# mickeyjoe666/PHFPFAC

Measured on AMD Instinct MI355X. Metric: input GB/s scanned, higher is better.
Workload: dtype u8

## Files before the change

phfpfac_amd/csrc/pfac_hip.hip:

```cpp
#include <hip/hip_runtime.h>
#include <hip/hip_ext.h>

#include <stdint.h>
#include <stdio.h>
#include <stdlib.h>
#include <string.h>

#include <algorithm>
#include <mutex>
#include <type_traits>
#include <string>
#include <vector>

#include "pfac.h"

namespace {

constexpr int WAVE = 64;
constexpr int SUB = WAVE * 16;
constexpr int SUBS = 4;
constexpr int WTILE = SUB * SUBS;
constexpr int MSUBS = 2;
constexpr int MSUB = WTILE / MSUBS;
constexpr int MLANE = MSUB / WAVE;
constexpr int HALO_MAX = 1024;
constexpr int QCAP = SUB / 2 + 4 * WAVE;
#ifndef PFAC_CAPW
#define PFAC_CAPW 256
#endif
constexpr int CAPW = PFAC_CAPW;
constexpr int PACK_STATE_BITS = 20;
constexpr int MAX_WAVES_PER_BLOCK = 16;
constexpr int LDS_TOTAL = 160 * 1024;
constexpr int LDS_TABLE_MAX = 40 * 1024;

constexpr int SH_HDR = 0;
constexpr int SH_S0 = SH_HDR + 2048;
constexpr int SH_FTAB = SH_S0 + 256 * 4;
constexpr int SH_D1IDX = SH_FTAB + 4 * 256;
constexpr int SH_FIN = SH_D1IDX + 256;
constexpr int SH_COLMAP = SH_FIN + 256;
constexpr int SH_D1 = SH_COLMAP + 256;
constexpr int D1_LDS_MAX = 32 * 1024;
constexpr int D1_STATE_BITS = 20;
constexpr int D1_N2_MAX = 2048;
#ifndef PFAC_L2F_UNROLL
#define PFAC_L2F_UNROLL 1
#endif
constexpr int L2F_UNROLL = PFAC_L2F_UNROLL;
#ifndef PFAC_MASK_GATHERS
#define PFAC_MASK_GATHERS 1
#endif
constexpr bool MASK_GATHERS = PFAC_MASK_GATHERS != 0;
#ifndef PFAC_LOAD_AUX
#define PFAC_LOAD_AUX 2
#endif
constexpr int LOAD_AUX = PFAC_LOAD_AUX;
#ifndef PFAC_PAIR_DENSITY_PCT
#define PFAC_PAIR_DENSITY_PCT 40
#endif
constexpr int QDEEP = 0x8000;
constexpr int NBUF_MAX = 3;
constexpr int CAPW3_MIN = 192;
constexpr int PW_FIXED_1BUF = WTILE + QCAP * 2;
constexpr int CAPW_DENSE = 2048;
constexpr int PW_FIXED_DENSE = PW_FIXED_1BUF + CAPW_DENSE * 4;
constexpr int D2_RING = 256;
constexpr int D2_CNT_OFF = D2_RING * 8;
constexpr int D2_PREF_OFF = D2_CNT_OFF + WTILE / 2;
constexpr int D2_AUX = D2_PREF_OFF + (WTILE / 8) * 2;
static_assert(D2_AUX >= QCAP * 2 && D2_AUX % 16 == 0, "the survivor FIFO of the fallback pass lies in the same bytes");
constexpr int PW_FIXED_DENSE2 = WTILE + D2_AUX;
constexpr unsigned D2_LOG_CAP = 4096;

#ifndef PFAC_TICKET_WAYS
#define PFAC_TICKET_WAYS 4
#endif
constexpr unsigned TICKET_WAYS = PFAC_TICKET_WAYS;
constexpr unsigned CTL_WORDS = 64u * (TICKET_WAYS + 1);
constexpr unsigned SPIN_MAX = 1u << 22;
constexpr unsigned CTL_ERR = 32, CTL_OVF = 33, CTL_DONE = 34, CTL_OVF2 = 35, CTL_TOTAL = 36 ;
constexpr unsigned CTL_CURSOR = 64u * TICKET_WAYS;

typedef unsigned int u32x4 __attribute__((ext_vector_type(4)));

struct ScanArgs {
    const unsigned char *in;
    unsigned long long n_owned, n_avail;
    void *out;
    unsigned long long out_cap;
    unsigned long long *tile_index;
    unsigned chunk;
    unsigned rec_bytes;
    const int *s0;
    const int *r;
    const int2 *T;
    const int4 *T4;
    int r_words, t_entries;
    int ht_size, wbit, num_final, halo;
    int rn_bias;
    int shared_bytes, pw_bytes;
    const int *d1;
    const unsigned char *d1idx;
    const unsigned char *d1_colmap;
    const unsigned char *d1_colbyte;
    int d1_rows;
    int d1_stride, d1_ncols, d1_lds_bytes;
    const int2 *d1r2;
    int d1_n2;
    unsigned root_byte;
    int root_state;
    int l2f_mode;
    unsigned child0, child1;
// ... 228 lines not shown
    };
    if (!reached(1, false)) return;
    if (dense1) {
        unsigned col[NWALK];
        int nx[NWALK];
#pragma unroll
        for (int w = 0; w < NWALK; w++) col[w] = colmap[(win[w] >> 8) & 0xFFu];
#pragma unroll
        for (int w = 0; w < NWALK; w++) nx[w] = D1[(go[w] ? f[w] : 0u) * d1_stride + col[w]];
        if (FUSED && D1R2) {
            bool ok[NWALK];
            int2 e2[NWALK];
#pragma unroll
            for (int w = 0; w < NWALK; w++) {
                ok[w] = go[w] && nx[w] >= 0;
                e2[w] = D1R2[ok[w] ? (nx[w] >> D1_STATE_BITS) : 0];
            }
#pragma unroll
            for (int w = 0; w < NWALK; w++) {
                s[w] = ok[w] ? (nx[w] & ((1 << D1_STATE_BITS) - 1)) : -1;
                rn[w] = e2[w].x;
                cm[w] = (unsigned)e2[w].y;
            }
        } else {
#pragma unroll
            for (int w = 0; w < NWALK; w++) s[w] = go[w] ? nx[w] : -1;
        }
        k++;
    } else {
        if (FUSED && S0R) {
#pragma unroll
            for (int w = 0; w < NWALK; w++) rn[w] = S0R[win[w] & 0xFFu];
        } else {
            load_rn();
        }
        step(1);
    }
    if (!reached(2, true)) return;
    if (dense1 && !(FUSED && D1R2)) load_rn();
    step(2);
    if (!reached(3, true)) return;
    step(3);
    for (;;) {
        if (!reached(0, false)) return;
#pragma unroll
        for (int w = 0; w < NWALK; w++) {
            const unsigned p = pos[w] + 1u + k;
            const unsigned lo = t32[p >> 2], hi = t32[(p >> 2) + 1];
            win[w] = __builtin_amdgcn_alignbyte(hi, lo, p & 3u);
        }
        if (USE_CM) {
            bool any = false;
#pragma unroll
            for (int w = 0; w < NWALK; w++) {
                go[w] = go[w] && ((cm[w] >> (win[w] & 31u)) & 1u) != 0u;
                any = any || go[w];
            }
            if (!__any(any)) return;
        }
        step(0);
        if (!reached(1, true)) return;
        step(1);
        if (!reached(2, true)) return;
        step(2);
        if (!reached(3, true)) return;
        step(3);
    }
}

__device__ __forceinline__ void put_record(const ScanArgs &a, unsigned long long ri, unsigned tpos, unsigned gpos, unsigned state) {
    if (ri >= a.out_cap) return;
    if (a.rec_bytes == 2) {
        static_cast<unsigned short *>(a.out)[ri] = (unsigned short)(tpos | (state << 12));
    } else if (a.rec_bytes == 4) {
        static_cast<unsigned *>(a.out)[ri] = tpos | (state << 12);
    } else {
        pfac_record rec;
        rec.pos = gpos;
        rec.state = state;
        static_cast<pfac_record *>(a.out)[ri] = rec;
    }
}

template <bool W8, bool DIRECT>
__device__ __forceinline__ void walk_store(const ScanArgs &a, const unsigned char *tile, const int *s0, const int *R, const int2 *T,
                                           unsigned pos, unsigned lim, unsigned *stage, unsigned long long ri, unsigned gpos) {
    unsigned n = 0;
    int s = s0[tile[pos]];
    unsigned p = pos + 1;
    while (s >= 0) {
        if (s < a.num_final) {
            if (DIRECT) put_record(a, ri + n, pos, gpos, (unsigned)s);
            else if (ri + n < a.stage_cap) stage[ri + n] = pos | ((unsigned)s << 12);
            n++;
        }
        if (p >= lim) break;
        s = phf_step<W8>(R, T, s, tile[p], a.wbit, a.ht_size);
        p++;
    }
}

struct Dense1 {
    const unsigned char *colmap;
    const unsigned char *idx;
    const int *rows;
    bool on;
    const int2 *r2;
    const int *s0r;
};

template <bool W8, bool DIRECT, int NWALK, bool FUSED, int ROOT>
__device__ __forceinline__ unsigned roundN(const ScanArgs &a, const unsigned char *tile, const int *s0, const Dense1 &d1,
                                           const int *R, const int2 *T, const unsigned short *q, unsigned q0,
                                           unsigned nact, int lane, unsigned *stage, unsigned lim,
                                           unsigned long long tile_base, unsigned long long wrun) {
    static_assert(NWALK >= 1 && NWALK <= 4, "one to four walks per lane");
    constexpr int MREG = NWALK == 4 ? 4 : 2;
    bool active[NWALK], deepf[NWALK];
    unsigned pos[NWALK], n[NWALK], m[NWALK][MREG];
    bool anydeep = false;
#pragma unroll
    for (int w = 0; w < NWALK; w++) {
        active[w] = (unsigned)lane + WAVE * w < nact;
        const unsigned e = active[w] ? q[q0 + WAVE * w + lane] : 0u;
        pos[w] = e & 0xFFFu;
        deepf[w] = (e & QDEEP) != 0;
        anydeep = anydeep || deepf[w];
    }
#ifdef PFAC_ABL_NOWALK
    anydeep = false;
#endif
    if (!__any(anydeep)) {
#pragma unroll
        for (int w = 0; w < NWALK; w++) {
            if (!active[w]) continue;
            const unsigned st = ROOT == 1 ? (unsigned)a.root_state : (unsigned)s0[tile[pos[w]]];
            const unsigned long long ri = wrun + WAVE * w + lane;
            if (DIRECT) put_record(a, ri, pos[w], (unsigned)tile_base + pos[w], st);
            else if (ri < a.stage_cap) stage[ri] = pos[w] | (st << 12);
        }
        return nact;
    }
    walkN<W8, NWALK, FUSED, MREG, ROOT>(tile, s0, a.root_state, d1.idx, d1.colmap, (unsigned)a.d1_stride, d1.rows, d1.on, d1.r2, d1.s0r, R, T, a.T4, pos, active, deepf, lim,
                                        a.wbit, a.ht_size, a.num_final, a.rn_bias, ROOT != 1 && d1.on && a.sec_filter != 0, n, m);
#pragma unroll
    for (int w = 0; w < NWALK; w++) {
        const unsigned c = n[w];
        if (MREG == 4) {
            const unsigned a0 = m[w][0], a1 = m[w][1], a2 = m[w][2], a3 = m[w][3];
            m[w][0] = c >= 4u ? a3 : (c == 3u ? a2 : (c == 2u ? a1 : a0));
            m[w][1] = c >= 4u ? a2 : (c == 3u ? a1 : a0);
            m[w][2] = c >= 4u ? a1 : a0;
            m[w][3] = a0;
        } else {
            const unsigned a0 = m[w][0], a1 = m[w][1];
            m[w][0] = c >= 2u ? a1 : a0;
            m[w][1] = a0;
        }
    }
    unsigned ex[NWALK], total = 0;
#pragma unroll
    for (int w0 = 0; w0 < NWALK; w0 += 2) {
        const bool pair = w0 + 1 < NWALK;
        const unsigned packed = pair ? (n[w0] | (n[pair ? w0 + 1 : w0] << 16)) : n[w0];
        const unsigned inc = wave_incl_scan(packed);
        const unsigned last = bcast_last(inc);
        const unsigned t0 = pair ? (last & 0xFFFFu) : last;
        ex[w0] = total + (pair ? (inc & 0xFFFFu) : inc) - n[w0];
        total += t0;
        if (pair) {
            ex[w0 + 1] = total + (inc >> 16) - n[w0 + 1];
            total += last >> 16;
        }
    }
#pragma unroll
    for (int w = 0; w < NWALK; w++) {
        const bool regs = n[w] <= (unsigned)MREG;
        const unsigned gpos = (unsigned)tile_base + pos[w];
        if (DIRECT) {
            const unsigned long long ri = wrun + ex[w];
            if (regs && n[w] > 0) put_record(a, ri, pos[w], gpos, m[w][0]);
#pragma unroll
            for (int k = 1; k < MREG; k++)
                if (regs && n[w] > (unsigned)k) put_record(a, ri + k, pos[w], gpos, m[w][k]);
            if (!regs) walk_store<W8, true>(a, tile, s0, R, T, pos[w], lim, nullptr, ri, gpos);
        } else {
            const unsigned ri = (unsigned)wrun + ex[w];
            if (regs && n[w] > 0 && ri < a.stage_cap) stage[ri] = pos[w] | (m[w][0] << 12);
#pragma unroll
            for (int k = 1; k < MREG; k++)
                if (regs && n[w] > (unsigned)k && ri + k < a.stage_cap) stage[ri + k] = pos[w] | (m[w][k] << 12);
            if (!regs) walk_store<W8, false>(a, tile, s0, R, T, pos[w], lim, stage, ri, 0);
        }
    }
    return total;
}

template <bool W8, bool DIRECT, int NWALK, bool FUSED, int ROOT>
__device__ __forceinline__ unsigned long long tile_pass(const ScanArgs &a, const unsigned char *tile, const int *s0,
                                                        const Dense1 &d1, const int *R, const int2 *T, unsigned short *q,
                                                        unsigned *stage, const unsigned (&keep)[MSUBS],
                                                        const unsigned (&deep)[MSUBS], int lane,
                                                        unsigned lim, unsigned long long tile_base,
                                                        unsigned long long wrun) {
    unsigned head = 0, tail = 0;
    static_assert(MSUBS == 2, "the packed scan assumes 2 half-tiles");
    const unsigned c0 = __popc(keep[0]), c1 = __popc(keep[1]);
    const unsigned pa = wave_incl_scan(c0 | (c1 << 16));
    const unsigned incls[MSUBS] = {pa & 0xFFFFu, pa >> 16};
    const unsigned cnts[MSUBS] = {c0, c1};
    const unsigned la = bcast_last(pa);
    const unsigned totals[MSUBS] = {la & 0xFFFFu, la >> 16};
    if (ROOT == 1 && !__any((deep[0] | deep[1]) != 0u)) {
        const unsigned st = (unsigned)a.root_state;
#pragma unroll
        for (int j = 0; j < MSUBS; j++) {
            if (totals[j] == 0) continue;
            const unsigned lpos = j * MSUB + lane * MLANE;
            unsigned o = (j ? totals[0] : 0u) + incls[j] - cnts[j];
#ifdef PFAC_ABL_NOSTAGE
            if (true) continue;
#endif
            if (!DIRECT && totals[0] + totals[1] <= a.stage_cap) {
                const unsigned w0 = lpos | (st << 12);
                for (unsigned m = keep[j]; m;) {
                    stage[o] = w0 + (unsigned)__ffs(m) - 1u;
                    m &= m - 1;
                    if (m) stage[o + 1] = w0 + (unsigned)__ffs(m) - 1u;
                    m &= m - 1;
                    o += 2;
                }
                continue;
            }
            for (unsigned m = keep[j]; m; m &= m - 1) {
                const unsigned pos = lpos + (__ffs(m) - 1);
                if (DIRECT) put_record(a, wrun + o, pos, (unsigned)tile_base + pos, st);
                else if (o < a.stage_cap) stage[o] = pos | (st << 12);
                o++;
            }
        }
        return wrun + totals[0] + totals[1];
    }
    constexpr unsigned RW = WAVE * NWALK;
#ifdef PFAC_TRACE_BUILD
    unsigned long long tp_round = 0, tp_n = 0, tp_t0 = __builtin_amdgcn_s_memrealtime();
#define TP_ROUND(call) do { const unsigned long long t_ = __builtin_amdgcn_s_memrealtime(); call; tp_round += __builtin_amdgcn_s_memrealtime() - t_; tp_n++; } while (0)
#else
#define TP_ROUND(call) do { call; } while (0)
#endif
#pragma unroll
    for (int j = 0; j < MSUBS; j++) {
        const unsigned mask = keep[j];
        const unsigned dmask = deep[j];
        const unsigned cnt = cnts[j];
        const unsigned incl = incls[j];
        const unsigned S = totals[j];
        if (S == 0) continue;
        const unsigned lpos = j * MSUB + lane * MLANE;
        const int ngrp = S > 512u ? 4 : 1;
        for (int gi = 0; gi < ngrp; gi++) {
            unsigned gbase = 0, gcnt = S;
            bool mine = true;
            if (ngrp != 1) {
                gbase = gi ? __builtin_amdgcn_readlane(incl, 16 * gi - 1) : 0u;
                gcnt = __builtin_amdgcn_readlane(incl, 16 * gi + 15) - gbase;
                mine = (lane >> 4) == gi;
            }
            if (tail + gcnt > (unsigned)QCAP) {
                const unsigned rem = tail - head;
                unsigned short v[NWALK];
#pragma unroll
                for (int w = 0; w < NWALK; w++) v[w] = (unsigned)lane + WAVE * w < rem ? q[head + WAVE * w + lane] : (unsigned short)0;
                wave_lds_sync();
#pragma unroll
                for (int w = 0; w < NWALK; w++) if ((unsigned)lane + WAVE * w < rem) q[WAVE * w + lane] = v[w];
                head = 0;
                tail = rem;
            }
            if (mine) {
                unsigned o = tail + (incl - cnt) - gbase;
                for (unsigned m = mask; m; m &= m - 1) {
                    const unsigned b = __ffs(m) - 1;
                    q[o++] = (unsigned short)((lpos + b) | (((dmask >> b) & 1u) << 15));
                }
            }
            tail += gcnt;
            wave_lds_sync();
            for (; head + RW <= tail; head += RW)
                TP_ROUND((wrun += roundN<W8, DIRECT, NWALK, FUSED, ROOT>(a, tile, s0, d1, R, T, q, head, RW, lane, stage, lim, tile_base, wrun)));
        }
    }
    if (tail > head) {
        if (NWALK == 2 && !DIRECT && tail - head <= (unsigned)WAVE)
            TP_ROUND((wrun += roundN<W8, DIRECT, 1, FUSED, ROOT>(a, tile, s0, d1, R, T, q, head, tail - head, lane, stage, lim, tile_base, wrun)));
        else
            TP_ROUND((wrun += roundN<W8, DIRECT, NWALK, FUSED, ROOT>(a, tile, s0, d1, R, T, q, head, tail - head, lane, stage, lim, tile_base, wrun)));
    }
#ifdef PFAC_TRACE_BUILD
    if (!DIRECT && a.dbg && blockIdx.x < 8 && lane == 0 && (threadIdx.x >> 6) == 0) {
        unsigned long long *acc = a.dbg + (size_t)blockIdx.x * 64 * 32 + 10;
        acc[0] += tp_round; acc[1] += tp_n; acc[2] += __builtin_amdgcn_s_memrealtime() - tp_t0; acc[3] += 1; acc[4] += tail - head;
    }
#endif
    return wrun;
}

template <bool SPARSE>
__device__ __forceinline__ void copy_out(const ScanArgs &a, const unsigned *stage, unsigned cnt, unsigned long long base, int lane) {
    if (cnt == 0) return;
#ifdef PFAC_ABL_NOEMIT
    return;
#endif
    if (a.rec_bytes == 2) {
        unsigned short *out = static_cast<unsigned short *>(a.out);
        if (base + cnt > a.out_cap) {
            for (unsigned i = (unsigned)lane; i < cnt; i += WAVE)
                if (base + i < a.out_cap) out[base + i] = (unsigned short)stage[i];
            return;
        }
        unsigned head = (0u - (unsigned)base) & 7u;
        head = head < cnt ? head : cnt;
        if ((unsigned)lane < head) out[base + lane] = (unsigned short)stage[lane];
        unsigned i = head + 8u * (unsigned)lane;
        for (; i + 8u <= cnt; i += 8u * WAVE) {
            const u32x4 v = {(stage[i] & 0xFFFFu) | (stage[i + 1] << 16), (stage[i + 2] & 0xFFFFu) | (stage[i + 3] << 16),
                             (stage[i + 4] & 0xFFFFu) | (stage[i + 5] << 16), (stage[i + 6] & 0xFFFFu) | (stage[i + 7] << 16)};
            __builtin_nontemporal_store(v, reinterpret_cast<u32x4 *>(out + base + i));
        }
        const unsigned tail = head + ((cnt - head) & ~7u);
        if (tail + (unsigned)lane < cnt) out[base + tail + lane] = (unsigned short)stage[tail + lane];
        return;
    }
    if (SPARSE && cnt <= 2u * WAVE && base + cnt <= a.out_cap) {
        unsigned *out = static_cast<unsigned *>(a.out);
        const unsigned v0 = (unsigned)lane < cnt ? stage[lane] : 0u, v1 = (unsigned)lane + WAVE < cnt ? stage[lane + WAVE] : 0u;
        if ((unsigned)lane < cnt) __builtin_nontemporal_store(v0, out + base + lane);
        if ((unsigned)lane + WAVE < cnt) __builtin_nontemporal_store(v1, out + base + lane + WAVE);
        return;
    }
    unsigned *out = static_cast<unsigned *>(a.out);
    if (base + cnt > a.out_cap) {
        for (unsigned i = (unsigned)lane; i < cnt; i += WAVE)
            if (base + i < a.out_cap) out[base + i] = stage[i];
        return;
    }
    unsigned head = (0u - (unsigned)base) & 3u;
    head = head < cnt ? head : cnt;
    if ((unsigned)lane < head) out[base + lane] = stage[lane];
    unsigned i = head + 4u * (unsigned)lane;
    for (; i + 4u <= cnt; i += 4u * WAVE) {
        const u32x4 v = {stage[i], stage[i + 1], stage[i + 2], stage[i + 3]};
        __builtin_nontemporal_store(v, reinterpret_cast<u32x4 *>(out + base + i));
    }
    const unsigned tail = head + ((cnt - head) & ~3u);
    if (tail + (unsigned)lane < cnt) out[base + tail + lane] = stage[tail + lane];
}

#ifndef PFAC_D2_FB
#define PFAC_D2_FB 2
#endif
#ifndef PFAC_D2_NS
#define PFAC_D2_NS 2
#endif
constexpr int D2_FB = PFAC_D2_FB;
static_assert(D2_RING >= (D2_FB + 1) * WAVE, "ring: one trip's pushes on top of a batch of left-overs");
template <bool W8>
__device__ __forceinline__ unsigned dense2_tile(const ScanArgs &a, const unsigned char *tile, const unsigned *t0, const Dense1 &d1,
                                                unsigned char *aux, unsigned *logg, int lane, unsigned lim, unsigned own_end) {
    constexpr int NS = PFAC_D2_NS;
    uint2 *ring = reinterpret_cast<uint2 *>(aux);
    const unsigned *t32 = reinterpret_cast<const unsigned *>(tile);
    const int sub = a.wbit - 8;
    const unsigned nfin = (unsigned)a.num_final, logcap = a.d2log_cap;
    const __amdgpu_buffer_rsrc_t lrs = __builtin_amdgcn_make_buffer_rsrc(logg, 0, (int)(logcap * 4u), 0x00020000);
    unsigned pos[NS], pn[NS], jn[NS];
    int s[NS], idx[NS];
    bool alive[NS];
#pragma unroll
    for (int w = 0; w < NS; w++) { pos[w] = pn[w] = jn[w] = 0u; s[w] = -1; idx[w] = 0; alive[w] = false; }
    unsigned P0 = 0, head = 0, fcount = 0, lc = 0;
    unsigned jmax = 0;
    const unsigned no_root = 0xFFFFu | ((unsigned)(a.d1_rows * a.d1_stride) << 16);
    auto lane_rank = [&](unsigned long long b) -> unsigned {
        return __builtin_amdgcn_mbcnt_hi((unsigned)(b >> 32), __builtin_amdgcn_mbcnt_lo((unsigned)b, 0u));
    };
    unsigned *stg = reinterpret_cast<unsigned *>(aux + D2_CNT_OFF);
    constexpr unsigned STG = (unsigned)(WTILE / 2 / 4);
    static_assert(STG >= (unsigned)(WAVE + 2 * D2_FB * WAVE) && STG >= (unsigned)(WAVE + PFAC_D2_NS * WAVE), "log staging: < 64 words pending + what a trip / a step adds");
    unsigned fl = 0;
    auto log_put = [&](bool f, unsigned word) {
        const unsigned long long b = __builtin_amdgcn_ballot_w64(f);
        if (b) {
            if (f) stg[(lc + lane_rank(b)) & (STG - 1u)] = word;
            lc += (unsigned)__popcll(b);
        }
// ... 329 lines not shown
        for (int i = tid; i < 256; i += blockDim.x) { d1idx_l[i] = 0; colmap_l[i] = 0; }
    }
    if (a.d1_rows > 0)
        for (int i = tid; i < a.d1_stride; i += blockDim.x) d1_l[a.d1_rows * a.d1_stride + i] = -1;
    const unsigned *t0_l = reinterpret_cast<const unsigned *>(smem + a.sh_t0);
    if (FUSED && NW == 4 && a.sh_t0)
        for (int i = tid; i < 256; i += blockDim.x) {
            const int v = a.s0[i];
            reinterpret_cast<unsigned *>(smem + a.sh_t0)[i] = v >= 0 ? (((unsigned)v < (unsigned)a.num_final ? (unsigned)v : 0xFFFFu) | ((unsigned)(a.d1idx[i] * a.d1_stride) << 16))
                                                                     : (0xFFFFu | ((unsigned)(a.d1_rows * a.d1_stride) << 16));
        }
    int2 *d1r2_l = reinterpret_cast<int2 *>(smem + SH_D1 + a.d1_lds_bytes);
    if (FUSED && a.d1_n2 > 0)
        for (int i = tid; i <= a.d1_n2; i += blockDim.x) {
            const int2 e = i < a.d1_n2 ? a.d1r2[i] : make_int2(-a.rn_bias, 0);
            d1r2_l[i] = make_int2(e.x + a.rn_bias, e.y);
        }
    int *s0r_l = reinterpret_cast<int *>(smem + SH_D1);
    const bool have_s0r = FUSED && a.d1_rows == 0;
    if (have_s0r)
        for (int i = tid; i < 256; i += blockDim.x) {
            const int v = a.s0[i];
            s0r_l[i] = v >= 0 ? a.r[v >> (a.wbit - 8)] + a.rn_bias : 0;
        }
    const Dense1 d1 = {colmap_l, d1idx_l, d1_l, a.d1_rows > 0, (FUSED && a.d1_n2 > 0) ? d1r2_l : nullptr, have_s0r ? s0r_l : nullptr};
    const int sh_tab = SH_D1 + a.d1_lds_bytes;
    const int *R = a.r;
    const int2 *T = a.T;
    if (TLDS) {
        int *lr = reinterpret_cast<int *>(smem + sh_tab);
        int2 *lt = reinterpret_cast<int2 *>(smem + sh_tab + ((a.r_words * 4 + 15) & ~15));
        for (int i = tid; i < a.r_words; i += blockDim.x) lr[i] = a.r[i];
        for (int i = tid; i < a.t_entries; i += blockDim.x) lt[i] = a.T[i];
        R = lr;
        T = lt;
    }
    const unsigned char *bm2l = smem + a.sh_bm2;
    if (a.l2f_mode == 2) {
        const unsigned *src = reinterpret_cast<const unsigned *>(a.bm2 + (ROOT == 1 ? (a.root_byte & 0xFFu) * 32u : 0u));
        unsigned *dst = reinterpret_cast<unsigned *>(smem + a.sh_bm2);
        for (int i = tid; i < a.bm2_rows * 8; i += blockDim.x) dst[i] = src[i];
    }
    __syncthreads();
#ifdef PFAC_TRACE_BUILD
    if (a.dbg && blockIdx.x < 8 && threadIdx.x == 0) a.dbg[((size_t)blockIdx.x * 64 + 1) * 32 + 15] = __builtin_amdgcn_s_memrealtime();
#endif

#ifdef PFAC_ABL_NOCOORD
    if (wave == nc) return;
#endif
    if (wave == nc) {
        __builtin_amdgcn_s_setprio(3);
#ifdef PFAC_ABL_STATIC
        unsigned abl_seq = 0;
        auto ticket = [&]() -> unsigned { return (abl_seq++) * gridDim.x + blockIdx.x; };
#else
        auto ticket = [&]() -> unsigned {
            unsigned g = 0;
            if (lane == 0) g = atomicAdd(&a.ctl[(blockIdx.x % a.ticket_ways) * 64u], 1u) * a.ticket_ways + blockIdx.x % a.ticket_ways;
            return g;
        };
#endif
        auto publish_batch = [&](unsigned r, unsigned g_lane0) -> unsigned {
            if (lane == 0) {
                lds_store(&hdr[H_ARRIVED + (r & 7)], 0u);
                lds_store(&hdr[H_BATCH + (r & 7)], g_lane0);
                __builtin_amdgcn_fence(__ATOMIC_RELEASE, "workgroup");
                lds_store(&hdr[H_EPOCH + (r & 7)], r + 1);
            }
            return __builtin_amdgcn_readfirstlane(g_lane0);
        };
        unsigned g[AHEAD];
#pragma unroll
        for (int k = 0; k < AHEAD; k++) g[k] = publish_batch((unsigned)k, ticket());
        unsigned t_pending = ticket();
        unsigned long long *cursor = reinterpret_cast<unsigned long long *>(a.ctl + CTL_CURSOR);
        auto order_chunk = [&]() -> unsigned long long {
            unsigned long long v = 0;
            if (lane == 0 && a.chunk) v = __hip_atomic_fetch_add(cursor, (unsigned long long)a.chunk, __ATOMIC_RELAXED, __HIP_MEMORY_SCOPE_AGENT);
            return v;
        };
        unsigned long long ch_base = 0, spare = order_chunk(), local_total = 0;
        unsigned ch_size = 0, ch_used = 0;
        for (unsigned r = 0;; r++) {
            const unsigned g_cur = g[0];
            const unsigned long long first = (unsigned long long)g_cur * (unsigned)nc;
            if (first >= a.n_tiles) break;
            const unsigned g_new = publish_batch(r + AHEAD, t_pending);
            t_pending = ticket();
#ifdef PFAC_TRACE_BUILD
            const bool trace = a.dbg && blockIdx.x < 8 && r < 64 && lane == 0;
            unsigned long long *tr = a.dbg + ((size_t)blockIdx.x * 64 + (r & 63)) * 32;
#endif
            PFAC_STAMP(trace, 0);
            const unsigned long long left = a.n_tiles - first;
            const unsigned n_valid = left < (unsigned long long)nc ? (unsigned)left : (unsigned)nc;
            if (!lds_wait_eq(&hdr[H_ARRIVED + (r & 7)], n_valid, err, 4u)) break;
            PFAC_STAMP(trace, 1);
            const unsigned c_raw = (unsigned)lane < n_valid ? hdr[H_CNT + (r & 7) * 16 + lane] : 0u;
            const unsigned c_all = c_raw & 0x7FFFFFFFu;
            const bool self_placed = (c_raw >> 31) != 0u;
            const unsigned c = self_placed ? 0u : c_all;
            const unsigned incl = wave_incl_scan(c);
            const unsigned tot = bcast_last(incl);
            const unsigned excl = incl - c;
            const unsigned tot_all = __any(self_placed) ? bcast_last(wave_incl_scan(c_all)) : tot;
            unsigned long long wb;
            if (tot == 0) {
                wb = ch_base + ch_used;
            } else if (tot > a.chunk) {
                unsigned long long v = 0;
                if (lane == 0) v = __hip_atomic_fetch_add(cursor, (unsigned long long)tot, __ATOMIC_RELAXED, __HIP_MEMORY_SCOPE_AGENT);
                const unsigned lo = __builtin_amdgcn_readfirstlane((unsigned)v), hi = __builtin_amdgcn_readfirstlane((unsigned)(v >> 32));
                wb = (((unsigned long long)hi << 32) | lo) + excl;
            } else if (ch_used + tot <= ch_size) {
                wb = ch_base + ch_used + excl;
                ch_used += tot;
            } else {
                const unsigned long long fits = __ballot(ch_used + incl <= ch_size);
                const unsigned k = (unsigned)__popcll(fits);
                const unsigned off = __builtin_amdgcn_readlane(excl, k);
                const unsigned lo = __builtin_amdgcn_readfirstlane((unsigned)spare), hi = __builtin_amdgcn_readfirstlane((unsigned)(spare >> 32));
                const unsigned long long nb = ((unsigned long long)hi << 32) | lo;
                wb = (unsigned)lane < k ? ch_base + ch_used + excl : nb + (excl - off);
                ch_base = nb;
                ch_size = a.chunk;
                ch_used = tot - off;
                spare = order_chunk();
            }
            local_total += tot_all;
            const bool mute = (a.fault & 1u) && blockIdx.x == 1 && r == 1;
            if (lane < nc) {
                hdr[H_WBASE + (r & 7) * 32 + lane * 2] = (unsigned)wb;
                hdr[H_WBASE + (r & 7) * 32 + lane * 2 + 1] = (unsigned)(wb >> 32);
            }
            __builtin_amdgcn_fence(__ATOMIC_RELEASE, "workgroup");
            if (lane == 0 && !mute) lds_store(&hdr[H_READY + (r & 7)], r + 1);
            if ((unsigned)lane < n_valid && !self_placed) a.tile_index[first + (unsigned)lane] = wb | ((unsigned long long)c << TIX_CNT_SHIFT);
#ifdef PFAC_TRACE_BUILD
            if (trace) { tr[2] = __builtin_amdgcn_s_memrealtime(); tr[3] = g_cur; }
#endif
#pragma unroll
            for (int k = 0; k + 1 < AHEAD; k++) g[k] = g[k + 1];
            g[AHEAD - 1] = g_new;
        }
        if (lane == 0) {
            if (local_total) __hip_atomic_fetch_add(reinterpret_cast<unsigned long long *>(a.ctl + CTL_TOTAL), local_total, __ATOMIC_RELAXED, __HIP_MEMORY_SCOPE_AGENT);
            const unsigned ovf = lds_load(&hdr[H_OVF]);
            if (ovf) __hip_atomic_fetch_add(&a.ctl[CTL_OVF], ovf, __ATOMIC_RELAXED, __HIP_MEMORY_SCOPE_AGENT);
            const unsigned ovf2 = lds_load(&hdr[H_OVF2]);
            if (ovf2) __hip_atomic_fetch_add(&a.ctl[CTL_OVF2], ovf2, __ATOMIC_RELAXED, __HIP_MEMORY_SCOPE_AGENT);
        }
        return;
    }

    unsigned char *tile = smem + a.shared_bytes + wave * a.pw_bytes;
    unsigned short *q = reinterpret_cast<unsigned short *>(tile + WTILE + a.halo);
    const bool d2 = NW == 4 && FUSED && a.dense2 != 0;
    unsigned char *aux = tile + WTILE + a.halo;
    unsigned *stage0 = reinterpret_cast<unsigned *>(aux + QCAP * 2);
    unsigned *d2log = d2 ? a.d2log + ((size_t)blockIdx.x * (unsigned)nc + (unsigned)wave) * a.d2log_cap : nullptr;
    const bool root_final = ROOT == 1 && (unsigned)a.root_state < (unsigned)a.num_final;

    u32x4 wA[SUBS], wB[SUBS];
    u32x4 hA = {0u, 0u, 0u, 0u}, hB = {0u, 0u, 0u, 0u};
    auto issue_loads = [&](unsigned long long tt, u32x4 (&w)[SUBS], u32x4 &hw) {
        const unsigned long long tb = tt * WTILE;
        const unsigned long long remain = a.n_avail - tb;
        const unsigned lm = remain < (unsigned long long)(WTILE + a.halo) ? (unsigned)remain : (unsigned)(WTILE + a.halo);
        const __amdgpu_buffer_rsrc_t rsrc = __builtin_amdgcn_make_buffer_rsrc(
            const_cast<unsigned char *>(a.in + tb), 0, (int)(lm & ~15u), 0x00020000);
#pragma unroll
        for (int j = 0; j < SUBS; j++) w[j] = __builtin_amdgcn_raw_buffer_load_b128(rsrc, j * SUB + lane * 16, 0, LOAD_AUX);
        if (lane * 16 < a.halo) hw = __builtin_amdgcn_raw_buffer_load_b128(rsrc, WTILE + lane * 16, 0, 0);
    };
    auto probe = [&](unsigned rr, unsigned long long &tt) -> bool {
#ifdef PFAC_ABL_NOCOORD
        tt = ((unsigned long long)rr * gridDim.x + blockIdx.x) * (unsigned)nc + (unsigned)wave;
        return tt < a.n_tiles;
#endif
        if (!lds_wait_eq(&hdr[H_EPOCH + (rr & 7)], rr + 1, err, 16u)) return false;
        tt = (unsigned long long)__builtin_amdgcn_readfirstlane(hdr[H_BATCH + (rr & 7)]) * (unsigned)nc + (unsigned)wave;
        return tt < a.n_tiles;
    };
    auto record_base = [&](unsigned rr, unsigned long long &base) -> bool {
        if (!lds_wait_eq(&hdr[H_READY + (rr & 7)], rr + 1, err, 8u)) return false;
        const unsigned blo = __builtin_amdgcn_readfirstlane(hdr[H_WBASE + (rr & 7) * 32 + wave * 2]);
        const unsigned bhi = __builtin_amdgcn_readfirstlane(hdr[H_WBASE + (rr & 7) * 32 + wave * 2 + 1]);
        base = ((unsigned long long)bhi << 32) | blo;
        return true;
    };

    unsigned r = 0;
    unsigned long long t = 0, t_n1 = 0;
    bool have_n1 = false;
    if (!probe(0, t)) return;
    issue_loads(t, wA, hA);
    if (LOAD_DEPTH == 2) {
        have_n1 = probe(1, t_n1);
        if (have_n1) issue_loads(t_n1, wB, hB);
    }

    constexpr int LAG_MAX = NB - 1;
    const unsigned nbuf = NB == 3 ? 3u : a.nbuf;
    const unsigned lag = NB == 3 ? 2u : a.nbuf - 1u;
    bool pend_have[LAG_MAX];
    unsigned pend_cnt[LAG_MAX], buf = 0;
#pragma unroll
    for (int k = 0; k < LAG_MAX; k++) { pend_have[k] = false; pend_cnt[k] = 0; }

    auto round_body = [&](u32x4 (&w)[SUBS], u32x4 &hw) -> bool {
        const unsigned long long tile_base = t * WTILE;
        const unsigned long long remain = a.n_avail - tile_base;
        const unsigned lim = remain < (unsigned long long)(WTILE + a.halo) ? (unsigned)remain : (unsigned)(WTILE + a.halo);

#ifdef PFAC_TRACE_BUILD
        const bool trace = a.dbg && blockIdx.x < 8 && r < 64 && lane == 0 && wave == 0;
        unsigned long long *tr = a.dbg + ((size_t)blockIdx.x * 64 + (r & 63)) * 32;
#endif
        PFAC_STAMP(trace, 4);
#ifndef PFAC_ABL_NOLDSCOPY
// ... 74 lines not shown
                deep[j] = m1 & nextc;
                keep[j] = root_final ? m1 : deep[j];
            } else {
                unsigned dm = 0, fm = 0;
                const unsigned *t32 = reinterpret_cast<const unsigned *>(tile);
                unsigned cand = m1;
                if (ROOT != 1 && a.sec_filter) {
                    const unsigned nx = *reinterpret_cast<const unsigned *>(tile + off + 32);
                    const unsigned s32 = ((unsigned)ftab[nx & 0xFFu] >> 4) & 1u;
                    cand = m1 & ((((rlo >> 16) | (rhi & 0xFFFF0000u)) >> 1) | (s32 << 31));
                }
#ifdef PFAC_ABL_NOCLASS
                cand = 0;
#endif
                if (ROOT != 1 && a.l2f_mode == 3) {
                    dm = cand;
                    cand = 0;
                }
                for (unsigned mm = cand; mm;) {
                    unsigned b[L2F_UNROLL], win[L2F_UNROLL], v[L2F_UNROLL], fin[L2F_UNROLL];
                    bool on[L2F_UNROLL];
#pragma unroll
                    for (int u = 0; u < L2F_UNROLL; u++) {
                        on[u] = mm != 0u;
                        b[u] = on[u] ? (unsigned)__ffs(mm) - 1u : 0u;
                        mm &= mm - 1u;
                        const unsigned p = off + b[u];
                        const unsigned lo = t32[p >> 2], hi = t32[(p >> 2) + 1];
                        win[u] = __builtin_amdgcn_alignbyte(hi, lo, p & 3u);
                    }
#pragma unroll
                    for (int u = 0; u < L2F_UNROLL; u++) {
                        const unsigned b0 = win[u] & 0xFFu, b1 = (win[u] >> 8) & 0xFFu;
                        v[u] = bm2l[(ROOT == 1 ? 0u : b0 * 32u) + (b1 >> 3)];
                        fin[u] = ROOT == 1 ? 0u : (unsigned)finl[b0];
                    }
#pragma unroll
                    for (int u = 0; u < L2F_UNROLL; u++) {
                        const unsigned b1 = (win[u] >> 8) & 0xFFu;
                        dm |= on[u] ? ((v[u] >> (b1 & 7u)) & 1u) << b[u] : 0u;
                        fm |= on[u] ? fin[u] << b[u] : 0u;
                    }
                }
                deep[j] = dm;
                keep[j] = dm | (ROOT == 1 ? (root_final ? m1 : 0u) : fm);
            }
#ifdef PFAC_TRACE_BUILD
            asm volatile("" :: "v"(keep[j]), "v"(deep[j]));
            PFAC_STAMP(trace && r > 0 && j == 0, 13);
#endif
        }
        }

#ifdef PFAC_ABL_NOKEEP
        asm volatile("" :: "v"(keep[0]), "v"(keep[1]), "v"(deep[0]), "v"(deep[1]));
        keep[0] = keep[1] = deep[0] = deep[1] = 0;
#endif
        PFAC_STAMP(trace, 6);
        const unsigned long long cnt = d2done ? (unsigned long long)d2cnt : !__any((keep[0] | keep[1]) != 0u) ? 0ull :
            tile_pass<W8, false, NW, FUSED, ROOT>(a, tile, s0, d1, R, T, q, stage, keep, deep, lane, lim, tile_base, 0);
        PFAC_STAMP(trace, 7);
#ifdef PFAC_TRACE_BUILD
        if (a.dbg && blockIdx.x < 8 && r < 64 && lane == 0) tr[16 + wave] = __builtin_amdgcn_s_memrealtime();
#endif
        const bool overflow = cnt > a.stage_cap;
        const bool now = overflow || nbuf == 1;
        unsigned arrival = 0;
#ifdef PFAC_ABL_NOCOORD
        if (false)
#endif
        if (lane == 0) {
            hdr[H_CNT + (r & 7) * 16 + wave] = (unsigned)cnt | ((now && cnt != 0) ? 0x80000000u : 0u);
            if (cnt > a.small_cap) {
                atomicAdd(&hdr[H_OVF2], 1u);
                if (cnt > a.sparse_cap) atomicAdd(&hdr[H_OVF], 1u);
            }
            __builtin_amdgcn_fence(__ATOMIC_RELEASE, "workgroup");
            arrival = atomicAdd(&hdr[H_ARRIVED + (r & 7)], 1u);
        }
        if (__builtin_amdgcn_readfirstlane(arrival) * 2u >= (unsigned)nc) __builtin_amdgcn_s_setprio(1);
        else __builtin_amdgcn_s_setprio(0);

        if (now && cnt != 0) {
            unsigned long long v = 0;
            if (lane == 0)
                v = __hip_atomic_fetch_add(reinterpret_cast<unsigned long long *>(a.ctl + CTL_CURSOR), (unsigned long long)cnt,
                                           __ATOMIC_RELAXED, __HIP_MEMORY_SCOPE_AGENT);
            const unsigned long long base = ((unsigned long long)__builtin_amdgcn_readfirstlane((unsigned)(v >> 32)) << 32) |
                                            __builtin_amdgcn_readfirstlane((unsigned)v);
            if (lane == 0) a.tile_index[t] = base | ((unsigned long long)cnt << TIX_CNT_SHIFT);
            PFAC_STAMP(trace && r > 0 && d2, 13);
            if (NW == 4 && FUSED && d2done) {
                dense2_scatter(a, aux, d2log, (unsigned)cnt, base, lane);
                PFAC_STAMP(trace && r > 0, 14);
            }
            else if (overflow)
                tile_pass<W8, true, NW, FUSED, ROOT>(a, tile, s0, d1, R, T, q, stage, keep, deep, lane, lim, tile_base, base);
            else
                copy_out<!TLDS>(a, stage, (unsigned)cnt, base, lane);
        }
        if (NB == 2) emit_pending(pend_have[0], pend_cnt[0]);
        PFAC_STAMP(trace, 8);
        if (NB == 3) { pend_have[LAG_MAX - 1] = pend_have[0]; pend_cnt[LAG_MAX - 1] = pend_cnt[0]; }
        pend_have[0] = !now; pend_cnt[0] = (unsigned)cnt;
        buf = buf + 1u >= nbuf ? 0u : buf + 1u;
        if (LOAD_DEPTH == 1) {
            if (!more_far) return false;
            t = t_far;
        } else {
            if (!have_n1) return false;
            t = t_n1;
            t_n1 = t_far;
            have_n1 = more_far;
        }
        r++;
        return true;
    };
    for (;;) {
        if (!round_body(wA, hA)) break;
        if (LOAD_DEPTH == 2 && !round_body(wB, hB)) break;
    }
#pragma unroll
    for (int k = LAG_MAX - 1; k >= 0; k--) {
        if ((unsigned)k < lag && pend_have[k] && pend_cnt[k] != 0) {
            unsigned long long base = 0;
            if (record_base(r - (unsigned)k, base))
                copy_out<!TLDS>(a, stage0 + ((buf + nbuf - 1u - (unsigned)k) % nbuf) * a.stage_cap, pend_cnt[k], base, lane);
        }
    }
}

template <bool TLDS, bool W8, int ROOT, bool FUSED, int NW, int NB = 2>
__global__ __launch_bounds__(WAVE * MAX_WAVES_PER_BLOCK) void pfac_scan_kernel(ScanArgs a) {
    static_assert(NB == 2 || (NB == 3 && NW <= 3), "three staging buffers: the sparse-mode kernels (dense mode has one)");
    static_assert(!(TLDS && FUSED), "the fused table is for tables gathered through L2");
    static_assert(NW == (TLDS ? 1 : 2) || (FUSED && (NW == 3 || NW == 4)), "walks per lane: 1 (LDS tables), 2 (L2 tables), 3 (L2, fused), 4 (L2, fused, dense matches)");
    extern __shared__ __attribute__((aligned(16))) unsigned char smem[];
    const ErrCh err = {&a.ctl[CTL_ERR], a.spin_max};
#ifdef PFAC_TRACE_BUILD
    if (a.dbg && blockIdx.x < 8 && threadIdx.x == 0) a.dbg[((size_t)blockIdx.x * 64 + 0) * 32 + 15] = __builtin_amdgcn_s_memrealtime();
#endif
    scan_body<TLDS, W8, ROOT, FUSED, NW, NB>(a, smem, err);
    unsigned *hdr = reinterpret_cast<unsigned *>(smem + SH_HDR);
    if ((threadIdx.x & (WAVE - 1)) == 0) {
        asm volatile("s_waitcnt vmcnt(0)" ::: "memory");
        const unsigned left = atomicAdd(&hdr[H_EXIT], 1u);
        if (left + 1 == (blockDim.x >> 6)) {
#ifdef PFAC_TRACE_BUILD
            if (a.dbg && blockIdx.x < 8) a.dbg[((size_t)blockIdx.x * 64 + 2) * 32 + 15] = __builtin_amdgcn_s_memrealtime();
#endif
            const unsigned done = __hip_atomic_fetch_add(&a.ctl[CTL_DONE], 1u, __ATOMIC_ACQ_REL, __HIP_MEMORY_SCOPE_AGENT);
            if (done + 1 == gridDim.x) {
                const unsigned long long tot = __hip_atomic_load(reinterpret_cast<unsigned long long *>(a.ctl + CTL_TOTAL), __ATOMIC_RELAXED, __HIP_MEMORY_SCOPE_AGENT);
                const unsigned long long cur = __hip_atomic_load(reinterpret_cast<unsigned long long *>(a.ctl + CTL_CURSOR), __ATOMIC_RELAXED, __HIP_MEMORY_SCOPE_AGENT);
                a.res[0] = (unsigned)tot; a.res[1] = (unsigned)(tot >> 32);
                a.res[2] = __hip_atomic_load(&a.ctl[CTL_ERR], __ATOMIC_RELAXED, __HIP_MEMORY_SCOPE_AGENT);
                a.res[3] = __hip_atomic_load(&a.ctl[CTL_OVF], __ATOMIC_RELAXED, __HIP_MEMORY_SCOPE_AGENT);
                a.res[4] = (unsigned)cur; a.res[5] = (unsigned)(cur >> 32);
                a.res[6] = __hip_atomic_load(&a.ctl[CTL_OVF2], __ATOMIC_RELAXED, __HIP_MEMORY_SCOPE_AGENT);
            }
        }
    }
}


__global__ void pfac_repack_kernel(const int *blob, int *s0, int *r, int2 *T, int *idmap, int max_row, int ht_size,
                                   int num_final, int state_num, int width, int *bad) {
    const int *b_s0 = blob + PFAC_BLOB_HEADER_WORDS;
    const int *b_r = b_s0 + 256;
// ... 1690 lines not shown
    const uint64_t n_tiles = (n_owned + WTILE - 1) / WTILE;
    if (s.pending) HIP_TRY(ctx, hipStreamSynchronize(s.stream));
    s.last_cap = capacity;
    s.scanned = true;
    s.pending = true;
    for (int i = 0; i < 7; i++) s.h_ctl[i] = 0;
    const bool dense = ctx->dense && ctx->stage_cap_d;
    const StageLayout &L = ctx->sparse();
    const int wpb = dense ? ctx->waves_per_block_d : L.waves_per_block;
    const int lds_bytes = dense ? ctx->lds_bytes_d : L.lds_bytes;
    s.last_dense = dense;
    s.last_tiles = n_tiles;
    s.last_owned = n_owned;
    s.last_avail = n_avail;
    s.scan_seq++;
    s.last_table = ctx->table_gen;
    s.last_rec_bytes = ctx->rec_bytes;
    s.last_records = d_records;
    rc = ensure_ctl(ctx, s);
    if (rc) return rc;
    rc = ensure_tiles(ctx, s, n_tiles + 1);
    if (rc) return rc;
    const uint64_t n_batches = (n_tiles + wpb - 2) / (wpb - 1);
    unsigned *const cur = s.d_ctlbuf[s.flip], *const nxt = s.d_ctlbuf[1 - s.flip];
    if (n_tiles > 0 && !s.clean[s.flip]) HIP_TRY(ctx, hipMemsetAsync(cur, 0, CTL_REGION, s.stream));
    if (n_tiles == 0) HIP_TRY(ctx, hipEventRecord(s.ev0, s.stream));
    if (n_tiles > 0) {
        ScanArgs a;
        a.in = in; a.n_owned = n_owned; a.n_avail = n_avail;
        a.out = d_records; a.out_cap = capacity;
        a.tile_index = s.d_tile_index;
        a.rec_bytes = (unsigned)ctx->rec_bytes;
        a.l2f_mode = ctx->l2f_mode; a.child0 = ctx->child0; a.child1 = ctx->child1; a.n_child = ctx->n_child;
        a.bm2 = ctx->d_bm2; a.bm2_rows = ctx->bm2_rows; a.sh_bm2 = ctx->sh_bm2; a.sh_t0 = ctx->sh_t0;
        a.sec2 = ctx->d_bm2 + 256 * 32; a.sec_filter = ctx->sec_filter;
        a.spin_max = ctx->spin_max; a.fault = ctx->fault;
        a.s0 = ctx->d_s0; a.r = ctx->d_r; a.T = ctx->d_T; a.T4 = ctx->d_T4_alloc; a.rn_bias = ctx->rn_bias;
        a.r_words = ctx->max_row; a.t_entries = ctx->ht_size;
        a.ht_size = ctx->ht_size; a.wbit = ctx->width_bit; a.num_final = ctx->num_final;
        a.halo = ctx->halo;
        a.shared_bytes = ctx->shared_bytes; a.pw_bytes = dense ? ctx->pw_bytes_d : L.pw_bytes;
        a.d1 = ctx->d_d1; a.d1_rows = ctx->d1_rows; a.d1_stride = ctx->d1_stride; a.d1_ncols = ctx->d1_ncols; a.d1_lds_bytes = ctx->d1_lds_bytes;
        a.d1_colmap = ctx->d_d1 ? reinterpret_cast<const unsigned char *>(ctx->d_d1) + d1_off_col(ctx->d1_rows) : nullptr;
        a.d1_colbyte = a.d1_colmap ? a.d1_colmap + 256 : nullptr;
        a.d1_n2 = ctx->d1_n2;
        a.d1r2 = ctx->d1_n2 ? reinterpret_cast<const int2 *>(reinterpret_cast<const unsigned char *>(ctx->d_d1) + d1_off_r2(ctx->d1_rows))
                            : nullptr;
        a.d1idx = ctx->d_d1 ? reinterpret_cast<const unsigned char *>(ctx->d_d1) + (size_t)ctx->d1_rows * 1024 : nullptr;
        a.root_byte = ctx->root_byte;
        a.root_state = ctx->root_state;
        a.stage_cap = dense ? ctx->stage_cap_d : L.stage_cap;
        a.nbuf = dense ? 1u : (unsigned)L.nbuf;
        a.dense2 = dense && ctx->dense2 ? 1 : 0;
        a.d2log = nullptr; a.d2log_cap = ctx->d2log_cap;
        if (a.dense2) {
            a.stage_cap = 0;
            const size_t words = (size_t)ctx->grid_blocks * (size_t)(wpb - 1) * ctx->d2log_cap;
            if (s.d2log_words < words) {
                if (s.d_d2log) { HIP_TRY(ctx, hipStreamSynchronize(s.stream)); HIP_TRY(ctx, hipFree(s.d_d2log)); s.d_d2log = nullptr; s.d2log_words = 0; }
                HIP_TRY(ctx, hipMalloc((void **)&s.d_d2log, words * 4));
                s.d2log_words = words;
            }
            a.d2log = s.d_d2log;
        }
        a.sparse_cap = ctx->lay[0].stage_cap;
        a.small_cap = ctx->lag2_ok ? ctx->lay[1].stage_cap : ctx->lay[0].stage_cap;
        a.n_tiles = (unsigned)n_tiles;
        a.ctl = cur;
        a.zero_next = reinterpret_cast<uint4 *>(nxt);
        a.zero_vec = (unsigned)(CTL_REGION / 16);
        a.res = s.d_res;
        a.dbg = nullptr;
#ifdef PFAC_TRACE_BUILD
        if (!ctx->trace_file.empty()) {
            if (!s.d_dbg) HIP_TRY(ctx, hipMalloc((void **)&s.d_dbg, 8 * 64 * 32 * 8));
            HIP_TRY(ctx, hipMemsetAsync(s.d_dbg, 0, 8 * 64 * 32 * 8, s.stream));
            a.dbg = s.d_dbg;
        }
#endif
        const uint64_t want = n_batches;
        uint64_t grid = (uint64_t)ctx->grid_blocks < want ? (uint64_t)ctx->grid_blocks : want;
        a.ticket_ways = grid < TICKET_WAYS ? (unsigned)grid : TICKET_WAYS;
        if (ctx->ticket_ways_knob >= 1 && ctx->ticket_ways_knob < a.ticket_ways) a.ticket_ways = ctx->ticket_ways_knob;
        uint64_t chunk = (capacity / (32 * grid)) & ~3ull;
        if (chunk > (1u << 22)) chunk = 1u << 22;
        a.chunk = (chunk >= 1024 && !dense) ? (unsigned)chunk : 0u;
        void *kargs[] = {&a};
        HIP_TRY(ctx, hipExtLaunchKernel(dense ? ctx->kernel_d : (ctx->lag2 ? ctx->kernel3 : ctx->kernel), dim3((unsigned)grid),
                                        dim3(WAVE * wpb), kargs, (size_t)lds_bytes, s.stream, s.ev0, s.ev1, 0));
        s.clean[s.flip] = false;
        s.clean[1 - s.flip] = true;
        s.flip = 1 - s.flip;
    }
    if (n_tiles == 0) HIP_TRY(ctx, hipEventRecord(s.ev1, s.stream));
    return PFAC_OK;
}

int pfac_scan_finish(pfac_ctx *ctx, int slot, uint64_t *n_matches) {
    int rc = check_slot(ctx, slot);
    if (rc) return rc;
    Slot &s = ctx->slots[slot];
    if (!s.scanned) return fail(ctx, PFAC_E_STATE, "pfac_scan_finish without a scan");
    USE_DEVICE(ctx);
    HIP_TRY(ctx, hipEventSynchronize(s.ev1));
    s.pending = false;
    const uint64_t total = ((uint64_t)s.h_ctl[1] << 32) | s.h_ctl[0];
    s.last_total = total;
    s.last_used = ((uint64_t)s.h_ctl[5] << 32) | s.h_ctl[4];
    if (n_matches) *n_matches = total;
#ifdef PFAC_TRACE_BUILD
    if (s.d_dbg && !ctx->trace_file.empty()) {
        std::vector<unsigned long long> h(8 * 64 * 32);
        if (hipMemcpy(h.data(), s.d_dbg, h.size() * 8, hipMemcpyDeviceToHost) == hipSuccess) {
            if (FILE *f = fopen(ctx->trace_file.c_str(), "wb")) { fwrite(h.data(), 8, h.size(), f); fclose(f); }
        }
    }
#endif
    if (s.h_ctl[2] != 0) {
        s.clean[0] = s.clean[1] = false;
        return fail(ctx, PFAC_E_INTERNAL, "scan kernel reported a timeout (flags " + std::to_string(s.h_ctl[2]) +
                                          ": 4 arrivals, 8 record base, 16 batch ring)");
    }
    if (ctx->dense_forced < 0 && ctx->stage_cap_d && s.last_tiles >= 64) {
        const uint64_t ovf = s.h_ctl[3];
        if (!ctx->dense && ovf * 4 > s.last_tiles) ctx->dense = true;
        else if (ctx->dense && ovf * 16 < s.last_tiles) ctx->dense = false;
    }
    if (ctx->lag2_ok && !ctx->lag_forced && s.last_tiles >= 64) {
        const uint64_t ovf2 = s.h_ctl[6];
        if (ctx->lag2 && ovf2 * 16 > s.last_tiles) ctx->lag2 = false;
        else if (!ctx->lag2 && ovf2 * 64 < s.last_tiles) ctx->lag2 = true;
    }
    if (s.last_used > s.last_cap)
        return fail(ctx, PFAC_E_OVERFLOW, "record array too small: " + std::to_string(total) + " matches need " +
                                              std::to_string(s.last_used) + " records of capacity (pfac_scan_capacity_hint)");
    return PFAC_OK;
}

int pfac_scan_elapsed_ms(pfac_ctx *ctx, int slot, float *ms) {
    int rc = check_slot(ctx, slot);
    if (rc) return rc;
    if (!ms) return fail(ctx, PFAC_E_ARG, "null argument");
    Slot &s = ctx->slots[slot];
    if (!s.scanned) return fail(ctx, PFAC_E_STATE, "no scan to time");
    HIP_TRY(ctx, hipEventSynchronize(s.ev1));
    HIP_TRY(ctx, hipEventElapsedTime(ms, s.ev0, s.ev1));
    return PFAC_OK;
}

static int ensure_gsum(pfac_ctx *ctx, Slot &s, unsigned n_groups) {
    if ((uint64_t)n_groups + 1 <= s.gsum_cap) return PFAC_OK;
    if (s.d_gsum) { HIP_TRY(ctx, hipStreamSynchronize(s.stream)); HIP_TRY(ctx, hipFree(s.d_gsum)); s.d_gsum = nullptr; }
    const uint64_t cap = n_groups < 4096 ? 4097 : (uint64_t)n_groups + n_groups / 4 + 1;
    HIP_TRY(ctx, hipMalloc((void **)&s.d_gsum, cap * 8));
    s.gsum_cap = cap;
    return PFAC_OK;
}

static int expand_records(pfac_ctx *ctx, Slot &s, const void *src, uint64_t first, uint64_t n, pfac_record *d_out) {
    if (s.pending) return fail(ctx, PFAC_E_STATE, "records requested before pfac_scan_finish");
    if (first + n > s.last_total) return fail(ctx, PFAC_E_ARG, "records [first, first + n) exceed the scan's match count");
    if (s.last_used > s.last_cap) return fail(ctx, PFAC_E_OVERFLOW, "the slot's last scan overflowed its record heap: scan again with a larger one");
    if (n == 0 || s.last_tiles == 0) return PFAC_OK;
    const unsigned n_groups = (unsigned)((s.last_tiles + XGROUP - 1) / XGROUP);
    int rc = ensure_gsum(ctx, s, n_groups);
    if (rc) return rc;
    const unsigned gblocks = (n_groups + 3) / 4;
// ... 673 lines not shown
```

Before: 4915.

## Stage 16-bit records in LDS and emit them with aligned 16-byte nontemporal stores

When the output record size is 2 bytes and the single-walk path is used, matches are staged in LDS as 16-bit values instead of 32-bit words. Each tile's output allocation is rounded up to a multiple of 8 records, so copy_out can write 8 records per lane with 16-byte nontemporal stores. The ticket/placement logic pads per-tile counts and keeps the true match totals separately. The aim is to cut LDS footprint and global store instructions for the output, at the cost of padding gaps in the output buffer and more complex count bookkeeping.

```diff
diff --git a/phfpfac_amd/csrc/pfac_hip.hip b/phfpfac_amd/csrc/pfac_hip.hip
--- a/phfpfac_amd/csrc/pfac_hip.hip
+++ b/phfpfac_amd/csrc/pfac_hip.hip
@@ -29,6 +29,7 @@
 #define PFAC_CAPW 256
 #endif
 constexpr int CAPW = PFAC_CAPW;
+static_assert(CAPW % 8 == 0, "staging buffers start on 16-byte boundaries (copy_out reads them 16 bytes per lane)");
 constexpr int PACK_STATE_BITS = 20;
 constexpr int MAX_WAVES_PER_BLOCK = 16;
 constexpr int LDS_TOTAL = 160 * 1024;
@@ -423,7 +424,13 @@
     }
 }
 
-template <bool W8, bool DIRECT>
+template <bool S16>
+__device__ __forceinline__ void stage_put(const ScanArgs &a, unsigned *stage, unsigned i, unsigned v) {
+    if (S16 && a.rec_bytes == 2) reinterpret_cast<unsigned short *>(stage)[i] = (unsigned short)v;
+    else stage[i] = v;
+}
+
+template <bool W8, bool DIRECT, bool S16>
 __device__ __forceinline__ void walk_store(const ScanArgs &a, const unsigned char *tile, const int *s0, const int *R, const int2 *T,
                                            unsigned pos, unsigned lim, unsigned *stage, unsigned long long ri, unsigned gpos) {
     unsigned n = 0;
@@ -432,7 +439,7 @@
     while (s >= 0) {
         if (s < a.num_final) {
             if (DIRECT) put_record(a, ri + n, pos, gpos, (unsigned)s);
-            else if (ri + n < a.stage_cap) stage[ri + n] = pos | ((unsigned)s << 12);
+            else if (ri + n < a.stage_cap) stage_put<S16>(a, stage, (unsigned)ri + n, pos | ((unsigned)s << 12));
             n++;
         }
         if (p >= lim) break;
@@ -450,7 +457,7 @@
     const int *s0r;
 };
 
-template <bool W8, bool DIRECT, int NWALK, bool FUSED, int ROOT>
+template <bool W8, bool DIRECT, int NWALK, bool FUSED, int ROOT, bool S16>
 __device__ __forceinline__ unsigned roundN(const ScanArgs &a, const unsigned char *tile, const int *s0, const Dense1 &d1,
                                            const int *R, const int2 *T, const unsigned short *q, unsigned q0,
                                            unsigned nact, int lane, unsigned *stage, unsigned lim,
@@ -478,7 +485,7 @@
             const unsigned st = ROOT == 1 ? (unsigned)a.root_state : (unsigned)s0[tile[pos[w]]];
             const unsigned long long ri = wrun + WAVE * w + lane;
             if (DIRECT) put_record(a, ri, pos[w], (unsigned)tile_base + pos[w], st);
-            else if (ri < a.stage_cap) stage[ri] = pos[w] | (st << 12);
+            else if (ri < a.stage_cap) stage_put<S16>(a, stage, (unsigned)ri, pos[w] | (st << 12));
         }
         return nact;
     }
@@ -524,14 +531,14 @@
 #pragma unroll
             for (int k = 1; k < MREG; k++)
                 if (regs && n[w] > (unsigned)k) put_record(a, ri + k, pos[w], gpos, m[w][k]);
-            if (!regs) walk_store<W8, true>(a, tile, s0, R, T, pos[w], lim, nullptr, ri, gpos);
+            if (!regs) walk_store<W8, true, S16>(a, tile, s0, R, T, pos[w], lim, nullptr, ri, gpos);
         } else {
             const unsigned ri = (unsigned)wrun + ex[w];
-            if (regs && n[w] > 0 && ri < a.stage_cap) stage[ri] = pos[w] | (m[w][0] << 12);
+            if (regs && n[w] > 0 && ri < a.stage_cap) stage_put<S16>(a, stage, ri, pos[w] | (m[w][0] << 12));
 #pragma unroll
             for (int k = 1; k < MREG; k++)
-                if (regs && n[w] > (unsigned)k && ri + k < a.stage_cap) stage[ri + k] = pos[w] | (m[w][k] << 12);
-            if (!regs) walk_store<W8, false>(a, tile, s0, R, T, pos[w], lim, stage, ri, 0);
+                if (regs && n[w] > (unsigned)k && ri + k < a.stage_cap) stage_put<S16>(a, stage, ri + k, pos[w] | (m[w][k] << 12));
+            if (!regs) walk_store<W8, false, S16>(a, tile, s0, R, T, pos[w], lim, stage, ri, 0);
         }
     }
     return total;
@@ -545,6 +552,7 @@
                                                         unsigned lim, unsigned long long tile_base,
                                                         unsigned long long wrun) {
     unsigned head = 0, tail = 0;
+    constexpr bool S16 = NWALK == 1;
     static_assert(MSUBS == 2, "the packed scan assumes 2 half-tiles");
     const unsigned c0 = __popc(keep[0]), c1 = __popc(keep[1]);
     const unsigned pa = wave_incl_scan(c0 | (c1 << 16));
@@ -564,6 +572,17 @@
 #endif
             if (!DIRECT && totals[0] + totals[1] <= a.stage_cap) {
                 const unsigned w0 = lpos | (st << 12);
+                if (S16 && a.rec_bytes == 2) {
+                    unsigned short *s16 = reinterpret_cast<unsigned short *>(stage);
+                    for (unsigned m = keep[j]; m;) {
+                        s16[o] = (unsigned short)(w0 + (unsigned)__ffs(m) - 1u);
+                        m &= m - 1;
+                        if (m) s16[o + 1] = (unsigned short)(w0 + (unsigned)__ffs(m) - 1u);
+                        m &= m - 1;
+                        o += 2;
+                    }
+                    continue;
+                }
                 for (unsigned m = keep[j]; m;) {
                     stage[o] = w0 + (unsigned)__ffs(m) - 1u;
                     m &= m - 1;
@@ -576,7 +595,7 @@
             for (unsigned m = keep[j]; m; m &= m - 1) {
                 const unsigned pos = lpos + (__ffs(m) - 1);
                 if (DIRECT) put_record(a, wrun + o, pos, (unsigned)tile_base + pos, st);
-                else if (o < a.stage_cap) stage[o] = pos | (st << 12);
+                else if (o < a.stage_cap) stage_put<S16>(a, stage, o, pos | (st << 12));
                 o++;
             }
         }
@@ -628,14 +647,14 @@
             tail += gcnt;
             wave_lds_sync();
             for (; head + RW <= tail; head += RW)
-                TP_ROUND((wrun += roundN<W8, DIRECT, NWALK, FUSED, ROOT>(a, tile, s0, d1, R, T, q, head, RW, lane, stage, lim, tile_base, wrun)));
+                TP_ROUND((wrun += roundN<W8, DIRECT, NWALK, FUSED, ROOT, S16>(a, tile, s0, d1, R, T, q, head, RW, lane, stage, lim, tile_base, wrun)));
         }
     }
     if (tail > head) {
         if (NWALK == 2 && !DIRECT && tail - head <= (unsigned)WAVE)
-            TP_ROUND((wrun += roundN<W8, DIRECT, 1, FUSED, ROOT>(a, tile, s0, d1, R, T, q, head, tail - head, lane, stage, lim, tile_base, wrun)));
+            TP_ROUND((wrun += roundN<W8, DIRECT, 1, FUSED, ROOT, S16>(a, tile, s0, d1, R, T, q, head, tail - head, lane, stage, lim, tile_base, wrun)));
         else
-            TP_ROUND((wrun += roundN<W8, DIRECT, NWALK, FUSED, ROOT>(a, tile, s0, d1, R, T, q, head, tail - head, lane, stage, lim, tile_base, wrun)));
+            TP_ROUND((wrun += roundN<W8, DIRECT, NWALK, FUSED, ROOT, S16>(a, tile, s0, d1, R, T, q, head, tail - head, lane, stage, lim, tile_base, wrun)));
     }
 #ifdef PFAC_TRACE_BUILD
     if (!DIRECT && a.dbg && blockIdx.x < 8 && lane == 0 && (threadIdx.x >> 6) == 0) {
@@ -652,6 +671,18 @@
 #ifdef PFAC_ABL_NOEMIT
     return;
 #endif
+    if (a.rec_bytes == 2 && !SPARSE) {
+        const unsigned short *s16 = reinterpret_cast<const unsigned short *>(stage);
+        unsigned short *out = static_cast<unsigned short *>(a.out);
+        if (((unsigned)base & 7u) != 0u || base + ((cnt + 7u) & ~7u) > a.out_cap) {
+            for (unsigned i = (unsigned)lane; i < cnt; i += WAVE)
+                if (base + i < a.out_cap) out[base + i] = s16[i];
+            return;
+        }
+        for (unsigned i = 8u * (unsigned)lane; i < cnt; i += 8u * WAVE)
+            __builtin_nontemporal_store(*reinterpret_cast<const u32x4 *>(s16 + i), reinterpret_cast<u32x4 *>(out + base + i));
+        return;
+    }
     if (a.rec_bytes == 2) {
         unsigned short *out = static_cast<unsigned short *>(a.out);
         if (base + cnt > a.out_cap) {
@@ -1147,6 +1178,7 @@
         };
         unsigned long long ch_base = 0, spare = order_chunk(), local_total = 0;
         unsigned ch_size = 0, ch_used = 0;
+        const unsigned rec_pad = a.rec_bytes == 2 ? 7u : 0u;
         for (unsigned r = 0;; r++) {
             const unsigned g_cur = g[0];
             const unsigned long long first = (unsigned long long)g_cur * (unsigned)nc;
@@ -1165,11 +1197,10 @@
             const unsigned c_raw = (unsigned)lane < n_valid ? hdr[H_CNT + (r & 7) * 16 + lane] : 0u;
             const unsigned c_all = c_raw & 0x7FFFFFFFu;
             const bool self_placed = (c_raw >> 31) != 0u;
-            const unsigned c = self_placed ? 0u : c_all;
+            const unsigned c = self_placed ? 0u : (c_all + rec_pad) & ~rec_pad;
             const unsigned incl = wave_incl_scan(c);
             const unsigned tot = bcast_last(incl);
             const unsigned excl = incl - c;
-            const unsigned tot_all = __any(self_placed) ? bcast_last(wave_incl_scan(c_all)) : tot;
             unsigned long long wb;
             if (tot == 0) {
                 wb = ch_base + ch_used;
@@ -1193,7 +1224,6 @@
                 ch_used = tot - off;
                 spare = order_chunk();
             }
-            local_total += tot_all;
             const bool mute = (a.fault & 1u) && blockIdx.x == 1 && r == 1;
             if (lane < nc) {
                 hdr[H_WBASE + (r & 7) * 32 + lane * 2] = (unsigned)wb;
@@ -1201,7 +1231,8 @@
             }
             __builtin_amdgcn_fence(__ATOMIC_RELEASE, "workgroup");
             if (lane == 0 && !mute) lds_store(&hdr[H_READY + (r & 7)], r + 1);
-            if ((unsigned)lane < n_valid && !self_placed) a.tile_index[first + (unsigned)lane] = wb | ((unsigned long long)c << TIX_CNT_SHIFT);
+            if ((unsigned)lane < n_valid && !self_placed) a.tile_index[first + (unsigned)lane] = wb | ((unsigned long long)c_all << TIX_CNT_SHIFT);
+            local_total += (rec_pad || __any(self_placed)) ? bcast_last(wave_incl_scan(c_all)) : tot;
 #ifdef PFAC_TRACE_BUILD
             if (trace) { tr[2] = __builtin_amdgcn_s_memrealtime(); tr[3] = g_cur; }
 #endif
@@ -1442,9 +1473,10 @@
         else __builtin_amdgcn_s_setprio(0);
 
         if (now && cnt != 0) {
+            const unsigned long long take = a.rec_bytes == 2 ? (cnt + 7ull) & ~7ull : cnt;
             unsigned long long v = 0;
             if (lane == 0)
-                v = __hip_atomic_fetch_add(reinterpret_cast<unsigned long long *>(a.ctl + CTL_CURSOR), (unsigned long long)cnt,
+                v = __hip_atomic_fetch_add(reinterpret_cast<unsigned long long *>(a.ctl + CTL_CURSOR), take,
                                            __ATOMIC_RELAXED, __HIP_MEMORY_SCOPE_AGENT);
             const unsigned long long base = ((unsigned long long)__builtin_amdgcn_readfirstlane((unsigned)(v >> 32)) << 32) |
                                             __builtin_amdgcn_readfirstlane((unsigned)v);
@@ -3301,7 +3333,7 @@
         uint64_t grid = (uint64_t)ctx->grid_blocks < want ? (uint64_t)ctx->grid_blocks : want;
         a.ticket_ways = grid < TICKET_WAYS ? (unsigned)grid : TICKET_WAYS;
         if (ctx->ticket_ways_knob >= 1 && ctx->ticket_ways_knob < a.ticket_ways) a.ticket_ways = ctx->ticket_ways_knob;
-        uint64_t chunk = (capacity / (32 * grid)) & ~3ull;
+        uint64_t chunk = (capacity / (32 * grid)) & ~7ull;
         if (chunk > (1u << 22)) chunk = 1u << 22;
         a.chunk = (chunk >= 1024 && !dense) ? (unsigned)chunk : 0u;
         void *kargs[] = {&a};
```

Result: faster. 5168 (median of 6 runs) (+5.1%).
